# jonnylaw/bayesian_dlms

Measured on AMD Instinct MI355X. Metric: Kalman filter+smooth series*timesteps/sec, higher is better.
Workload: dtype f64

## Files before the change

### bayesian_dlms_amd/_lib.py

```python
import ctypes
import os

HERE = os.path.dirname(os.path.abspath(__file__))
LIB_PATH = os.environ.get("DLM_ENGINE_LIB") or os.path.join(HERE, "libdlm_engine.so")

DLM_MEM_DEVICE, DLM_MEM_HOST = 0, 1
OPT_SMOOTHER_COMPAT_Q1 = 1 << 0
OPT_SVD_RAW_W_Q2 = 1 << 1
OPT_SVD_SAMPLER_Q9 = 1 << 2
OPT_FORCE_GENERIC = 1 << 3
OPT_STATS_OUTER = 1 << 4
OPT_ASYNC = 1 << 5
OPT_FFBS_SIMSMOOTH = 1 << 6
OPT_PACKED_SYM = 1 << 7
OPT_MODEL_UNCHANGED = 1 << 8
OPT_COUNT_STEPS = 1 << 9
OPT_TRUST_MODEL_UNCHANGED = 1 << 10
OPT_LOGLIK_LITERAL_Q7 = 1 << 11
OPT_STUDENTT_LITERAL = 1 << 12
OPT_NO_LANE = 1 << 16
OPT_NO_SAMPLER16 = 1 << 17
OPT_NO_WAVE = 1 << 18
OPT_FORCE_WAVE = 1 << 19
OPT_NO_SPARSE_F = 1 << 20
OPT_NO_SMALL_BATCH = 1 << 21
OPT_NO_STEADY = 1 << 22
OPT_NO_PIPE = 1 << 23
OPT_SHARED_COV = 1 << 24
OPT_SVD_PER_SERIES = 1 << 25
OPT_SAMPLER_PER_SERIES = 1 << 26
OPT_DRAW_EIG = 1 << 27
OPT_SMOOTHER_PER_SERIES = 1 << 28
OPT_NO_TABLE_REUSE = 1 << 29
OPT_TEST_FAIL_AFTER_TABLES = 1 << 30
# ... 107 lines not shown
```

### bayesian_dlms_amd/csrc/dlm_engine.hip

```cpp
#include "../../include/dlm_engine.h"
#include <cstdlib>
#include "dlm_internal.h"

#include <rccl/rccl.h>

#include <cstdio>
#include <cstring>
#include <set>
#include <string>
#include <vector>

using dlm::KArgs;

struct Workspace {
  void* p = nullptr;
  size_t bytes = 0;
  Workspace* next;
  explicit Workspace(Workspace*& list) : next(list) { list = this; }
};
template <class T>
struct Ws : Workspace {
  using Workspace::Workspace;
  operator T*() const { return (T*)p; }
};
// ... 420 lines not shown
int start_sampler_normals(dlm_engine* e, const KArgs& k, dlm::SampTabs& tb, bool big, hipEvent_t gate) {
  if (!k.z) {
    int rc = ensure(e, e->zws, big ? dlm::wave48_sampler_shared_normals_bytes(k) : dlm::sampler_shared_normals_bytes(k));
    if (rc) return rc;
    if (!e->rng_stream) {
      HIP_TRY(e, hipStreamCreateWithFlags(&e->rng_stream, hipStreamNonBlocking));
      HIP_TRY(e, hipEventCreateWithFlags(&e->rng_ev, hipEventDisableTiming));
    }
    if ((rc = aux_fork(e, e->rng_stream, e->rng_busy, gate, false))) return rc;
    if (big) HIP_TRY(e, dlm::launch_wave48_sampler_shared_normals(k, e->zws, e->rng_stream));
    else HIP_TRY(e, dlm::launch_sampler_shared_normals(k, e->zws, e->rng_stream));
    tb.z4 = e->zws;
  }
  return DLM_OK;
}
int start_rts_tables(dlm_engine* e, const KArgs& k, dlm::RtsTabs& tb) {
  bool fresh = false;
  int rc = ensure(e, e->rtsws, dlm::rts_shared_ws_bytes(k), &fresh);
  if (rc) return rc;
  if (fresh) HIP_TRY(e, hipMemsetAsync(e->rtsws, 0, 64, e->stream));
  if ((rc = ensure(e, e->covws, sizeof(double) * dlm::covtabs_doubles(k.d, k.T)))) return rc;
  if ((rc = ensure_route(e, (size_t)k.N)) || (rc = ensure_cov_stream(e))) return rc;
  dlm::RtsKeep keep{};
  dlm::rts_shared_carve(e->rtsws, k, tb, keep);
  dlm::CovTabs ctb{};
  dlm::covtabs_carve(e->covws, k.d, k.T, ctb);
  const bool no_reuse = (k.flags & DLM_OPT_NO_TABLE_REUSE) != 0;
  const int* gate = keep.ctl + dlm::RTS_CTL_GATE;
  e->rts_last = true;
  HIP_TRY(e, dlm::launch_rts_shared_mark(k, e->route, tb, e->stream));
  HIP_TRY(e, dlm::launch_rts_key_check(k, e->sparse_k, e->sp_dev, keep, no_reuse, e->stream));
  HIP_TRY(e, dlm::launch_rts_shared_cov(k, e->sparse_k, e->sp_dev, tb, ctb, gate, e->stream));
  if ((rc = aux_fork(e, e->cov_stream, e->cov_busy, e->cov_ev[0]))) return rc;
  HIP_TRY(e, dlm::launch_rts_shared_tables(k, e->sparse_k, e->sp_dev, tb, gate, e->cov_stream));
  HIP_TRY(e, dlm::launch_rts_key_commit(k, e->sparse_k, e->sp_dev, keep, no_reuse, e->cov_stream));
  return DLM_OK;
}
int ensure_shared(dlm_engine* e, const KArgs& k, dlm::CovTabs& tb, bool with_backward) {
  int rc = ensure(e, e->covws, sizeof(double) * dlm::covtabs_doubles(k.d, k.T));
  if (rc || (rc = ensure_route(e, (size_t)k.N)) || (rc = ensure_side(e, k.N, k.T)) || (rc = ensure_cov_stream(e))) return rc;
  dlm::covtabs_carve(e->covws, k.d, k.T, tb);
// ... 557 lines not shown
  if ((rc = st.commit())) return rc;
  if ((rc = analyse_g(e, k, model->G, opts->mem == DLM_MEM_HOST))) return rc;
  if (want_packed && (rc = packed_path(e, k))) return rc;
  bool fused_fast = fast_smoother_ok(e, k) || use_tiled(k);
  if (want_packed) k.packed = 3;
  const bool q1 = (k.flags & DLM_OPT_SMOOTHER_COMPAT_Q1) != 0;
  const bool rts_shared = fast_shape_ok(k) && e->sparse_k > 0 && !use_lane(k) && !k.packed && !(k.flags & DLM_OPT_SHARED_COV) &&
                          (q1 ? !fused_fast : fast_smoother_ok(e, k)) && dlm::rts_shared_eligible(k, !q1);
  if (!filt) {
    k.packed |= (fast_smoother_ok(e, k) && e->sparse_k > 0 && !use_lane(k) && !rts_shared) ? 1 : 0;
    if ((rc = ensure(e, e->fws, (k.packed & 1) ? N * (T + 1) * (size_t)dlm::packed_rec_bytes((int)d) : N * (T + 1) * rec * sizeof(double)))) return rc;
    k.filt = e->fws;
  }
  if ((rc = mark(e, 0))) return rc;
  dlm::RtsTabs rtb{};
  if (rts_shared && (rc = start_rts_tables(e, k, rtb))) return rc;
  if (rts_shared && (k.flags & DLM_OPT_TEST_FAIL_AFTER_TABLES))
    return fail(e, DLM_ERR_UNSUPPORTED, "DLM_OPT_TEST_FAIL_AFTER_TABLES");
  if ((rc = mark_plain(e, k))) return rc;
  if (filt && fast_smoother_ok(e, k) && use_shared_cov(e, k)) {
    dlm::CovTabs tb;
    if ((rc = run_shared_filter(e, k, tb, true))) return rc;
    if ((rc = mark(e, 1))) return rc;
    k.filt_in = k.filt;
    if ((rc = run_shared_smoother(e, k, tb))) return rc;
    if ((rc = mark(e, 2))) return rc;
    return st.finish(opts->flags & DLM_OPT_ASYNC);
  }
  if ((rc = run_filter(e, k, fused_fast))) return rc;
  if (rts_shared && (rc = join_cov(e))) return rc;
  if ((rc = mark(e, 1))) return rc;
  k.filt_in = k.filt;
  if (rts_shared) {
    k.route = e->route; k.route_take = 0;
    e->variant = "sparse16-rts-shared";
    HIP_TRY(e, dlm::launch_rts_shared_means(k, e->sparse_k, e->sp_dev, rtb, q1, e->stream));
    if (!q1) {
      KArgs kg = k;
      kg.route_take = 1;
      HIP_TRY(e, dlm::launch_sparse16_smoother(kg, e->sparse_k, e->sp_dev, e->side, e->stream));
    }
  } else if ((rc = run_smoother(e, k, fused_fast))) return rc;
  if ((rc = mark(e, 2))) return rc;
  return st.finish(opts->flags & DLM_OPT_ASYNC);
// ... 295 lines not shown
```

### bayesian_dlms_amd/csrc/dlm_internal.h

```cpp
#pragma once
#include <hip/hip_runtime.h>
#include <stdint.h>
#include <type_traits>

namespace dlm {

struct KArgs {
  int d, p, T, N;
  const double* F; long long f_stride;
  const double* G; int n_g; const int* g_index; const double* dt;
  const double* V; long long v_stride;
  const double* W; long long w_stride;
  long long v_tstride, w_tstride;
  const double* m0; long long m0_stride;
  const double* C0; long long c0_stride;
  const double* y;
  const double* z;
  const double* filt_in;
  double* filt;
  double* prior;
  double* fq;
  double* smooth;
  double* theta;
  double* cond;
// ... 68 lines not shown
hipError_t launch_sparse16_sampler(const KArgs& a, int K, const SparseT* tabs_dev, hipStream_t s);
hipError_t launch_small_mv_sampler(const KArgs& a, hipStream_t s);
hipError_t launch_sparse16_rts(const KArgs& a, int K, const SparseT* tabs_dev, hipStream_t s);
hipError_t launch_small_mv_rts(const KArgs& a, hipStream_t s);
hipError_t launch_sparse16_smoother(const KArgs& a, int K, const SparseT* cols_dev, const double* side, hipStream_t s);
hipError_t launch_sparse16_count_gaps(const KArgs& a, unsigned char* plain, hipStream_t s);
struct CovTabs {
  double* ftab;
  double* btab;
  double* cside;
  double* eq;
  double* mc;
  double* sc;
  int frow, brow;
  const int* skip;
};
size_t covtabs_doubles(int d, int T);
void covtabs_carve(double* base, int d, int T, CovTabs& t);
bool shared_cov_eligible(const KArgs& a);
hipError_t launch_sparse16_cov_filter(const KArgs& a, int K, const SparseT* rows_dev, const CovTabs& tabs, hipStream_t s);
hipError_t launch_sparse16_cov_smoother(const KArgs& a, int K, const SparseT* cols_dev, const CovTabs& tabs, hipStream_t s);
hipError_t launch_sparse16_mean_filter(const KArgs& a, int K, const SparseT* rows_dev, const CovTabs& tabs, hipStream_t s);
hipError_t launch_sparse16_mean_smoother(const KArgs& a, int K, const SparseT* cols_dev, const CovTabs& tabs, hipStream_t s);

struct SampTabs {
  double* rows;
  double* zrec;
  double* zeros;
  unsigned char* need;
  int* status;
  double* z4;
  int zstride;
  const double* mc4;
// ... 24 lines not shown
constexpr unsigned RTS_KEY_FLAGS = (1u << 0) | (1u << 22);
struct RtsKeySrc {
  int d, T, K;
  unsigned flags;
  const double *F, *V, *W, *C0;
  const SparseT* sp;
};
enum { RTS_CTL_HIT = 10,
       RTS_CTL_GATE = 11,
       RTS_CTL_VALID = 12,
       RTS_CTL_LAST = 13 };
struct RtsKeep { int* ctl; unsigned* key; };
constexpr int RTS_KEY_WORDS = 8 + 2 * (15 + 1 + 2 * 15 * 15) + 2 * (int)(sizeof(SparseT) / 4);
bool rts_shared_eligible(const KArgs& a, bool textbook);
size_t rts_shared_ws_bytes(const KArgs& a);
void rts_shared_carve(void* ws, const KArgs& a, RtsTabs& tb, RtsKeep& keep);
hipError_t launch_rts_key_check(const KArgs& a, int K, const SparseT* tabs_dev, const RtsKeep& keep, bool no_reuse, hipStream_t s);
hipError_t launch_rts_key_commit(const KArgs& a, int K, const SparseT* tabs_dev, const RtsKeep& keep, bool no_reuse, hipStream_t s);
hipError_t launch_rts_shared_cov(const KArgs& a, int K, const SparseT* tabs_dev, RtsTabs& tb, const CovTabs& ctb, const int* gate, hipStream_t s);
hipError_t launch_rts_shared_tables(const KArgs& a, int K, const SparseT* tabs_dev, const RtsTabs& tb, const int* gate, hipStream_t s);
hipError_t launch_rts_shared_mark(const KArgs& a, unsigned char* route, const RtsTabs& tb, hipStream_t s);
hipError_t launch_rts_shared_means(const KArgs& a, int K, const SparseT* tabs_dev, const RtsTabs& tb, bool own_rts, hipStream_t s);

bool wave48_sampler_shared_model_ok(const KArgs& a);
bool wave48_sampler_shared_eligible(const KArgs& a);
size_t wave48_sampler_shared_ws_bytes(const KArgs& a);
void wave48_sampler_shared_carve(void* ws, const KArgs& a, SampTabs& tb);
hipError_t launch_wave48_sampler_shared_tables(const KArgs& a, const SampTabs& tb, hipStream_t s, hipEvent_t after_filter = nullptr);
hipError_t launch_wave48_sampler_shared_draw(const KArgs& a, const SampTabs& tb, hipStream_t s);
size_t wave48_ktab_doubles(const KArgs& a);
hipError_t launch_wave48_steady_filter(const KArgs& a, const double* ktab, const int* settle, hipStream_t s);
// ... 159 lines not shown
```

### bayesian_dlms_amd/csrc/dlm_sampler16.hip

```cpp
#include "dlm_internal.h"
#include "dlm_wave.h"
#include "../../include/dlm_engine.h"

namespace dlm {
namespace s16 {

constexpr int IL = 17;
constexpr int IMG = 16 * IL;

__device__ __forceinline__ d4 mm(const d4& x, const d4& y, int rows) {
  d4 acc = {0.0, 0.0, 0.0, 0.0};
#pragma unroll
  for (int r = 0; r < 4; ++r)
    if (4 * r < rows) acc = __builtin_amdgcn_mfma_f64_16x16x4f64(x[r], y[r], acc, 0, 0, 0);
  return acc;
}
__device__ __forceinline__ void to_img(const d4& x, double* img, int g, int c) {
#pragma unroll
  for (int r = 0; r < 4; ++r) img[(4 * r + g) * IL + c] = x[r];
}
__device__ __forceinline__ d4 transposed(const d4& x, double* img, int g, int c) {
  to_img(x, img, g, c);
  wave_sync();
  d4 y;
// ... 1137 lines not shown
}

#ifndef DLM_RTS_SHARED_MIN
#define DLM_RTS_SHARED_MIN 2048
#endif
#ifndef DLM_RTS_SHARED_MIN_TEXTBOOK
#define DLM_RTS_SHARED_MIN_TEXTBOOK 6144
#endif
bool rts_shared_eligible(const KArgs& a, bool textbook) {
  return sampler_shared_model_ok(a) && a.y && !(a.flags & (DLM_OPT_FORCE_GENERIC | DLM_OPT_SMOOTHER_PER_SERIES | DLM_OPT_NO_STEADY)) &&
         (a.N >= (textbook ? DLM_RTS_SHARED_MIN_TEXTBOOK : DLM_RTS_SHARED_MIN) || (a.flags & DLM_OPT_NO_SMALL_BATCH));
}
static size_t rts_key_bytes() { return up64((size_t)RTS_KEY_WORDS * 4); }
size_t rts_shared_ws_bytes(const KArgs& a) {
  const size_t n1 = (size_t)a.T + 1, rec = (size_t)a.d + (size_t)a.d * a.d;
  return 64 + rts_key_bytes() + up64(n1 * s16::RJ_ROW * 8) + up64(n1 * rec * 8) + up64(n1);
}
void rts_shared_carve(void* ws, const KArgs& a, RtsTabs& tb, RtsKeep& keep) {
  const size_t n1 = (size_t)a.T + 1, rec = (size_t)a.d + (size_t)a.d * a.d;
  char* p = (char*)ws;
  keep.ctl = (int*)p; p += 64;
  keep.key = (unsigned*)p; p += rts_key_bytes();
  tb.jrows = (double*)p; p += up64(n1 * s16::RJ_ROW * 8);
  tb.srec = (double*)p;  p += up64(n1 * rec * 8);
  tb.need = (unsigned char*)p;
  tb.status = keep.ctl; tb.gaps = tb.status + 8; tb.skip = tb.status + 9;
  tb.crec = nullptr; tb.crec_stride = 0;
}
static RtsKeySrc rts_key_of(const KArgs& a, int K, const SparseT* tabs_dev) {
  RtsKeySrc s;
  s.d = a.d; s.T = a.T; s.K = K; s.flags = a.flags & RTS_KEY_FLAGS;
  s.F = a.F; s.V = a.V; s.W = a.W; s.C0 = a.C0; s.sp = tabs_dev;
  return s;
}
hipError_t launch_rts_key_check(const KArgs& a, int K, const SparseT* tabs_dev, const RtsKeep& keep, bool no_reuse, hipStream_t s) {
  if (a.d < 1 || a.d > 15) return hipErrorInvalidValue;
  return launch(s16::k_rts_key_check, dim3(1), dim3(256), 0, s, rts_key_of(a, K, tabs_dev), (const unsigned*)keep.key, keep.ctl, no_reuse ? 1 : 0);
}
hipError_t launch_rts_key_commit(const KArgs& a, int K, const SparseT* tabs_dev, const RtsKeep& keep, bool no_reuse, hipStream_t s) {
  if (a.d < 1 || a.d > 15) return hipErrorInvalidValue;
// ... 69 lines not shown
```

### bayesian_dlms_amd/csrc/dlm_sparse16.hip

```cpp
#include "dlm_internal.h"
#include "dlm_wave.h"
#include "../../include/dlm_engine.h"

namespace dlm {

constexpr int LD = 17;
constexpr int IMG = 16 * LD;
constexpr int WAVE_LDS = 2 * IMG + 8 * 16 + 2;

#ifndef DLM_SM_WAVES
#define DLM_SM_WAVES 4
#endif
#ifndef DLM_FI_WAVES
#define DLM_FI_WAVES 5
#endif
#ifndef DLM_SM_WAVES_K2
#define DLM_SM_WAVES_K2 5
#endif
constexpr int SM_WAVES_K2 = DLM_SM_WAVES_K2;
constexpr int SM_WAVES = DLM_SM_WAVES, FI_WAVES = DLM_FI_WAVES;

#ifdef DLM_STAMP
#define STAMP(k) { const unsigned long long _t = stamp(); seg[k] += _t - tlast; tlast = _t; }
#else
// ... 377 lines not shown
    } else {
      cc = R;
      steady = false;
      settle_reset(settle);
      bst128(rside, offS, (t + 1) * 16, __builtin_nan(""), __builtin_nan(""));
    }
    if (fq && lane == 0) { fq[2 * (t + 1)] = f; fq[2 * (t + 1) + 1] = Q; }
    const int so = (t + 1) * recb;
#pragma unroll
    for (int r = 0; r < 4; ++r) bst(rout, offA[r], so, cc[r]);
    wave_sync();
  }
  if (LL && a.loglik && lane == 0) a.loglik[n] = ll;
  if (!COV && a.counters && lane == 0) {
    if (nsteady) atomicAdd(&a.counters[0], (unsigned long long)nsteady);
    if (a.route) atomicAdd(&a.counters[3], 1ull);
  }
  bool bad = false;
#pragma unroll
  for (int r = 0; r < 4; ++r) bad |= va[r] && !isfinite(cc[r]);
  if (__ballot(bad) != 0ull) st |= DLM_ST_NONFINITE;
  if (a.status && lane == 0 && st) atomicOr(&a.status[n], st);
}

template <int K, bool SIM, bool IRR, bool LL = false>
__global__ __launch_bounds__(256, SIM ? 4 : FI_WAVES) void k_filter_sp16(KArgs a, const SparseT* __restrict__ sp,
                                                     double* __restrict__ side, double* __restrict__ xplus) {
  __shared__ __attribute__((aligned(16))) double lds[4 * WAVE_LDS + (SIM ? 4 * IMG : 0)];
  filter_body<K, SIM, IRR, LL>(a, sp, side, xplus, lds);
}
template <int K>
__global__ __launch_bounds__(64) void k_cov_filter_sp16(KArgs a, const SparseT* __restrict__ sp, double* __restrict__ side,
                                                        double* __restrict__ kftab, const int* __restrict__ skip) {
  if (skip && *skip) return;
  __shared__ __attribute__((aligned(16))) double lds[4 * WAVE_LDS];
  __builtin_amdgcn_s_setprio(3);
  filter_body<K, false, false, false, true>(a, sp, side, nullptr, lds, kftab);
}

__global__ __launch_bounds__(64) void k_cov_fill_sp16(double* __restrict__ ftab, int rowd, double* __restrict__ cside, const int* __restrict__ settle, int T) {
  const int t = blockIdx.x, ts = settle[0];
  if (t <= ts || t > T) return;
  const double* src = ftab + (size_t)ts * rowd;
  double* dst = ftab + (size_t)t * rowd;
  for (int i = threadIdx.x; i < rowd; i += 64) dst[i] = src[i];
  if (threadIdx.x < 2) cside[2 * (size_t)t + threadIdx.x] = cside[2 * (size_t)ts + threadIdx.x];
}

constexpr int SM_LDS = 2 * IMG + 3 * 16 + 2;
template <int K, bool IRR, bool PIPE = false, bool COV = false, bool PLAIN = false>
__device__ __forceinline__ void smoother_body(const KArgs& a, const SparseT* __restrict__ sp, const double* __restrict__ side,
                                              double* lds , char* ring_all, double* __restrict__ kbtab = nullptr) {
  const int lane = threadIdx.x & 63;
  const int wave = __builtin_amdgcn_readfirstlane(threadIdx.x >> 6);
  const int n = blockIdx.x * (int)(blockDim.x >> 6) + wave;
// ... 486 lines not shown
  if (__ballot(vc && !isfinite(thn)) != 0ull) st |= DLM_ST_NONFINITE;
  if (a.stats) {
    const int L = stats_len(d, 1, a.flags);
    double* sout = a.stats + (size_t)n * L;
    if (lane == 0) { sout[0] = ssy; sout[1] = nob; sout[L - 1] = (double)T; }
    if (outer) {
#pragma unroll
      for (int r = 0; r < 4; ++r) { const int i = 4 * r + g; if (i < d && vc) sout[2 + i + c * d] = so[r]; }
    } else if (g == 0 && vc) sout[2 + c] = ssc;
  }
  if (a.status && lane == 0 && st) atomicOr(&a.status[n], st);
}


constexpr int MEAN4_LDS = 6 * 64;
constexpr int MEAN_AHEAD = 8;

template <int K, int NP, int MODE>
__global__ __launch_bounds__(256) void k_mean_filter_sp16(KArgs a, const SparseT* __restrict__ sp, CovTabs tb) {
  constexpr bool REC = MODE != 0, CMP = MODE != 1;
  constexpr int NS = (REC ? NP : 0) + (CMP ? 1 : 0);
  __shared__ __attribute__((aligned(16))) double lds[4 * MEAN4_LDS];
  extern __shared__ __attribute__((aligned(16))) char ring_all[];
  const int lane = threadIdx.x & 63;
  const int wave = __builtin_amdgcn_readfirstlane(threadIdx.x >> 6);
  const int n0 = 4 * (blockIdx.x * (int)(blockDim.x >> 6) + wave);
  if (n0 >= a.N) return;
  const int j = lane >> 4, c = lane & 15;
  const int nser = a.N - n0 < 4 ? a.N - n0 : 4;
  const bool have = j < nser;
  const int n = have ? n0 + j : n0;
  double* vM = lds + wave * MEAN4_LDS;
  double* vW = vM + 64;
  double* vA = vW + 64;
  double* vH = vA + 64;
  const int d = a.d, T = a.T, rec = d + d * d, recb = rec * 8, frow = recb + 128;
  const bool vc = c < d;
  int idx[K];
  double val[K];
#pragma unroll
  for (int s = 0; s < K; ++s) { idx[s] = 16 * j + sp[0].idx[c][s]; val[s] = sp[0].val[c][s]; }
  const double V = a.V[0];
  const double* m0 = a.m0 + (size_t)n * a.m0_stride;
  const double* y = a.y + (size_t)n * T;
  const size_t sbytes = (size_t)(T + 1) * recb;
  char* bout = REC ? (char*)a.filt + (size_t)n0 * sbytes : nullptr;
  const __amdgpu_buffer_rsrc_t rout = mk_rsrc(bout, REC ? (size_t)nser * sbytes : 0);
  const __amdgpu_buffer_rsrc_t rcmp = mk_rsrc(CMP ? (char*)(tb.mc + (size_t)(n0 / 4) * (T + 1) * 64) : nullptr, CMP ? (size_t)(T + 1) * 512 : 0);
  const int offmc = have ? lane * 8 : OOB;
  double* eqn = tb.eq + (size_t)n * (T + 1);
  const double Fc = vc ? a.F[c] : 0.0;
  double F4[4];
#pragma unroll
  for (int k = 0; k < 4; ++k) F4[k] = ((c & 3) + 4 * k < d) ? a.F[(c & 3) + 4 * k] : 0.0;
  const int npc = rec / 2;
  unsigned psrc[NP];
  int pdst[NP], pser[NP];
#pragma unroll
  for (int k = 0; k < NP; ++k) {
    const int q = 64 * k + lane, sj = q / npc, pp = q - sj * npc;
    pser[k] = sj;
    pdst[k] = sj < nser ? (int)((size_t)sj * sbytes) + pp * 16 : OOB;
    psrc[k] = pp < 8 ? (0x80000000u | (unsigned)((16 * (sj & 3) + 2 * pp) * 8)) : (unsigned)(pp * 16);
  }
  const unsigned vH_lds = lds_addr_of(vH);
  char* ring = ring_all + wave * 2 * frow;
  const unsigned ring_lds = lds_addr_of(ring);
  const unsigned pkf = recb + c * 8, ptd = c * 8;
  const i4 rtab = rsrc_words(tb.ftab, (unsigned)((size_t)(T + 1) * frow));
  const int nrow = frow / 16;
  lds_dma<4>(rtab, ring_lds, 0, lane, nrow);
  lds_dma<4>(rtab, ring_lds + frow, frow, lane, nrow);
  double mcol = vc ? m0[c] : 0.0, mrow = mcol;
  int st = (V > 0.0) ? 0 : DLM_ST_NOT_PD;
  unsigned nsteady = 0;
  bool dead = !have;
  unsigned deadmask = (unsigned)(0xf << nser) & 0xf;
  vM[lane] = mcol; vW[lane] = mrow;
  double yk[4];
#pragma unroll
  for (int k = 0; k < 4; ++k) yk[k] = (16 * k + c < T) ? y[16 * k + c] : 0.0;
  asm volatile("" ::"v"(yk[0]), "v"(yk[1]), "v"(yk[2]), "v"(yk[3]));
  double ek[4] = {__builtin_nan(""), 0.0, 0.0, 0.0};
  wave_sync();
  vm_wait<1>();

  auto store = [&](const d2 (&pc)[NP], int so) {
#pragma unroll
    for (int k = 0; k < NP; ++k) bst128(rout, ((deadmask >> pser[k]) & 1u) ? OOB : pdst[k], so, pc[k]);
  };
  if constexpr (REC) {
    d2 pc[NP];
    {
      double td = lds_read64<0>(ring_lds + ptd);
      asm volatile("s_waitcnt lgkmcnt(0)" : "+v"(td)::"memory");
      vH[lane] = vc ? mcol : td;
      wave_sync();
#pragma unroll
      for (int k = 0; k < NP; ++k) pc[k] = lds_read128((psrc[k] & 0x80000000u) ? vH_lds + (psrc[k] & 0x7fffffffu) : ring_lds + psrc[k]);
      lds_wait<NP>(pc);
    }
    lds_dma<4>(rtab, ring_lds, (T >= 2 ? 2 : T) * frow, lane, nrow);
    store(pc, 0);
  } else lds_dma<4>(rtab, ring_lds, (T >= 2 ? 2 : T) * frow, lane, nrow);
  if constexpr (CMP) bst(rcmp, offmc, 0, vc ? mcol : 0.0);
  for (int t = 0; t < T; ++t) {
    if (t > 0 && (t & 63) == 0) {
#pragma unroll
      for (int k = 0; k < 4; ++k) yk[k] = (t + 16 * k + c < T) ? y[t + 16 * k + c] : 0.0;
      asm volatile("" ::"v"(yk[0]), "v"(yk[1]), "v"(yk[2]), "v"(yk[3]));
    }
    const int kk = (t >> 4) & 3;
    const double yt = row_pick(kk == 0 ? yk[0] : kk == 1 ? yk[1] : kk == 2 ? yk[2] : yk[3], lane, t & 15);
    if (!dead && !(yt == yt)) {
      dead = true;
      if (c == 0) a.route[n] = 1;
    }
    deadmask = 0;
#pragma unroll
    for (int q = 0; q < 4; ++q) deadmask |= (__builtin_amdgcn_readlane((int)dead, 16 * q) & 1) << q;
    if (deadmask == 0xfu) break;
    if (t == 0) vm_wait<NS + 1>(); else vm_wait<2 * NS + 1>();
    const unsigned slot = ring_lds + ((t + 1) & 1) * frow;
    double kfc = lds_read64<0>(slot + pkf);
    asm volatile("s_waitcnt lgkmcnt(0)" : "+v"(kfc)::"memory");
    const double rqs = readlane_d(kfc, 15);
    const double rq = fabs(rqs);
    double ac = vW[idx[0]] * val[0];
#pragma unroll
    for (int s = 1; s < K; ++s) ac = fma(vW[idx[s]], val[s], ac);
    double e, erq;
    if (rqs < 0.0) {
      nsteady += 4 - __builtin_popcount(deadmask);
      const double f = row_lane0(row_sum(Fc * ac), lane);
      e = yt - f; erq = e * rq;
      mcol = fma(kfc, e, ac);
      mrow = mcol;
    } else {
      double ar = vM[idx[0]] * val[0];
#pragma unroll
      for (int s = 1; s < K; ++s) ar = fma(vM[idx[s]], val[s], ar);
      vA[lane] = ac;
      wave_sync();
      double pf = 0.0;
#pragma unroll
      for (int k = 0; k < 4; ++k) pf = fma(vA[16 * j + (c & 3) + 4 * k], F4[k], pf);
      pf = pf + dpp_mov<0xB1>(pf);
      const double f = pf + dpp_mov<0x4E>(pf);
      e = yt - f; erq = e * rq;
      mcol = fma(kfc, erq, ac);
      mrow = fma(kfc * rq, e, ar);
    }
    {
      const int k1 = ((t + 1) >> 4) & 3;
      const bool mine = c == ((t + 1) & 15);
      ek[0] = (mine && k1 == 0) ? erq : ek[0]; ek[1] = (mine && k1 == 1) ? erq : ek[1];
      ek[2] = (mine && k1 == 2) ? erq : ek[2]; ek[3] = (mine && k1 == 3) ? erq : ek[3];
      if (((t + 1) & 63) == 63 || t + 1 == T) {
        const int base = (t + 1) & ~63;
#pragma unroll
        for (int k = 0; k < 4; ++k) if (!dead && base + 16 * k + c <= t + 1) eqn[base + 16 * k + c] = ek[k];
      }
    }
    wave_sync();
    vM[lane] = vc ? mcol : 0.0; vW[lane] = vc ? mrow : 0.0;
    wave_sync();
    if constexpr (REC) {
      d2 pc[NP];
      {
        double td = lds_read64<0>(slot + ptd);
        asm volatile("s_waitcnt lgkmcnt(0)" : "+v"(td)::"memory");
        vH[lane] = vc ? mcol : td;
        wave_sync();
#pragma unroll
        for (int k = 0; k < NP; ++k) pc[k] = lds_read128((psrc[k] & 0x80000000u) ? vH_lds + (psrc[k] & 0x7fffffffu) : slot + psrc[k]);
        lds_wait<NP>(pc);
      }
      { const int tn = t + 3 <= T ? t + 3 : T; lds_dma<4>(rtab, slot, tn * frow, lane, nrow); }
      store(pc, (t + 1) * recb);
    } else { const int tn = t + 3 <= T ? t + 3 : T; lds_dma<4>(rtab, slot, tn * frow, lane, nrow); }
    if constexpr (CMP) bst(rcmp, dead ? OOB : offmc, (t + 1) * 512, vc ? mcol : 0.0);
  }
  vm_wait<0>();
  if (have && !dead && c == 0) a.route[n] = 0;
  if (a.counters && lane == 0) { atomicAdd(&a.counters[2], (unsigned long long)(4 - __builtin_popcount(deadmask))); if (nsteady) atomicAdd(&a.counters[0], (unsigned long long)nsteady); }
  const unsigned long long badl = __ballot(!dead && vc && !isfinite(mcol));
  if (have && !dead && c == 0) {
    const int sj = st | (((badl >> (16 * j)) & 0xffffull) ? DLM_ST_NONFINITE : 0);
    if (a.status && sj) atomicOr(&a.status[n], sj);
  }
}

template <int K, int NP, bool REC>
__global__ __launch_bounds__(256) void k_mean_smoother_sp16(KArgs a, const SparseT* __restrict__ sp, CovTabs tb) {
  constexpr int NS = REC ? NP : 1;
  __shared__ __attribute__((aligned(16))) double lds[4 * MEAN4_LDS];
  extern __shared__ __attribute__((aligned(16))) char ring_all[];
  const int lane = threadIdx.x & 63;
  const int wave = __builtin_amdgcn_readfirstlane(threadIdx.x >> 6);
  const int n0 = 4 * (blockIdx.x * (int)(blockDim.x >> 6) + wave);
// ... 147 lines not shown
  }
  vm_wait<0>();
  if (a.counters && lane == 0 && nsteady) atomicAdd(&a.counters[1], (unsigned long long)nsteady);
  const unsigned long long badl = __ballot(!dead && vc && !isfinite(sm));
  if (!dead && c == 0) {
    const int sj = st | (((badl >> (16 * j)) & 0xffffull) ? DLM_ST_NONFINITE : 0);
    if (a.status && sj) atomicOr(&a.status[n], sj);
  }
}

size_t covtabs_doubles(int d, int T) { return (size_t)(T + 1) * (3 * (size_t)(d + d * d) + 16 + 16 + 2) + 64; }
void covtabs_carve(double* base, int d, int T, CovTabs& t) {
  const size_t rec = (size_t)(d + d * d), n1 = (size_t)T + 1;
  t.frow = (int)(rec * 8 + 128); t.brow = (int)(2 * rec * 8 + 128);
  t.ftab = base; t.btab = t.ftab + n1 * (rec + 16); t.cside = t.btab + n1 * (2 * rec + 16);
  t.skip = nullptr;
}
bool shared_cov_eligible(const KArgs& a) {
  return a.d <= 15 && a.p == 1 && !a.g_index && !a.dt && !a.f_stride && !a.v_tstride && !a.w_tstride && !a.v_stride && !a.w_stride &&
         !a.c0_stride && !a.packed && !a.prior && !a.fq && !a.loglik && a.filt && (a.flags & DLM_OPT_SHARED_COV) && !(a.flags & DLM_OPT_FORCE_GENERIC) &&
         4 * ((size_t)a.T + 1) * (size_t)(a.d + a.d * a.d) * 8 < ((size_t)1 << 31);
}

int sparse16_analyse(const double* G , int d, SparseT* rows, SparseT* cols) {
  int kmax = 1;
  for (int pass = 0; pass < 2; ++pass) {
    SparseT* t = pass ? cols : rows;
    for (int j = 0; j < 16; ++j)
      for (int s = 0; s < 4; ++s) { t->idx[j][s] = 0; t->val[j][s] = 0.0; }
    for (int j = 0; j < d; ++j) {
      int cnt = 0;
      for (int l = 0; l < d; ++l) {
        const double v = pass ? G[l + j * d]  : G[j + l * d] ;
        if (v != 0.0) {
          if (cnt == 4) return 99;
          t->idx[j][cnt] = l; t->val[j][cnt] = v; ++cnt;
// ... 57 lines not shown
}

hipError_t launch_sparse16_simsmooth(const KArgs& a, int K, const SparseT* tabs_dev, const double* side,
                                     const double* xplus, hipStream_t s) {
  return pick<1, 2, 3, 4>(K, [&](auto k) { return launch_ss<k()>(a, tabs_dev, side, xplus, s); });
}

static KArgs cov_args(const KArgs& a, const CovTabs& tb) {
  KArgs k = a;
  k.N = 1; k.y = nullptr; k.status = nullptr; k.route = nullptr; k.counters = nullptr; k.loglik = nullptr; k.prior = nullptr; k.fq = nullptr;
  k.filt = tb.ftab; k.filt_in = tb.ftab; k.smooth = tb.btab; k.packed = 0; k.m0_stride = 0; k.plain = nullptr;
  return k;
}
template <int K>
static hipError_t launch_cf(const KArgs& a, const SparseT* sp, const CovTabs& tb, hipStream_t s) {
  int* settle = (int*)(tb.cside + 2 * ((size_t)a.T + 1));
  hipError_t err = hipMemsetD32Async((hipDeviceptr_t)settle, a.T, 1, s);
  if (err != hipSuccess) return err;
  KArgs k = cov_args(a, tb);
  k.settle_step = (a.flags & DLM_OPT_NO_STEADY) ? nullptr : settle;
  if ((err = launch(k_cov_filter_sp16<K>, dim3(1), dim3(64), 0, s, k, sp, tb.cside, tb.ftab + (a.d + a.d * a.d), tb.skip)) != hipSuccess) return err;
  return launch(k_cov_fill_sp16, dim3(a.T + 1), dim3(64), 0, s, tb.ftab, tb.frow / 8, tb.cside, (const int*)settle, a.T);
}
template <int K>
static hipError_t launch_cs(const KArgs& a, const SparseT* sp, const CovTabs& tb, hipStream_t s) {
  const size_t ring = 2 * ((size_t)(a.d + a.d * a.d) * 8 + 16);
  return launch(k_cov_smoother_sp16<K>, dim3(1), dim3(64), ring, s, cov_args(a, tb), sp, (const double*)tb.cside, tb.btab);
}
template <class F>
static hipError_t with_mean_np(int d, F f) { return pick<4, 6, 8>(d <= 10 ? 4 : d <= 13 ? 6 : 8, f); }
template <int K>
static hipError_t launch_mf(const KArgs& a, const SparseT* sp, const CovTabs& tb, hipStream_t s) {
  const int wpb = a.N < 8192 ? 1 : 4, nw = (a.N + 3) / 4;
  const dim3 grid((nw + wpb - 1) / wpb), blk(64 * wpb);
  const size_t ring = (size_t)wpb * 2 * tb.frow;
  return pick<0, 2, 1>(tb.mc ? (a.filt ? 2 : 0) : 1, [&](auto MODE) {
    return with_mean_np(a.d, [&](auto NP) { return launch(k_mean_filter_sp16<K, NP(), decltype(MODE)::value>, grid, blk, ring, s, a, sp, tb); });
// ... 31 lines not shown
```

### include/dlm_engine.h

```cpp
#ifndef DLM_ENGINE_H
#define DLM_ENGINE_H

#include <stdint.h>

#ifdef __cplusplus
extern "C" {
#endif

typedef struct dlm_engine dlm_engine;

enum {
  DLM_OK = 0,
  DLM_ERR_ARG = -1,
  DLM_ERR_HIP = -2,
  DLM_ERR_UNSUPPORTED = -3,
  DLM_ERR_RCCL = -4
};

enum { DLM_MEM_DEVICE = 0, DLM_MEM_HOST = 1 };

enum {
  DLM_OPT_SMOOTHER_COMPAT_Q1 = 1u << 0,
  DLM_OPT_SVD_RAW_W_Q2 = 1u << 1,
  DLM_OPT_SVD_SAMPLER_Q9 = 1u << 2,
  DLM_OPT_FORCE_GENERIC = 1u << 3,
  DLM_OPT_STATS_OUTER = 1u << 4,
  DLM_OPT_ASYNC = 1u << 5,
  DLM_OPT_FFBS_SIMSMOOTH = 1u << 6,
  DLM_OPT_PACKED_SYM = 1u << 7,
  DLM_OPT_MODEL_UNCHANGED = 1u << 8,
  DLM_OPT_COUNT_STEPS = 1u << 9,
  DLM_OPT_TRUST_MODEL_UNCHANGED = 1u << 10,
  DLM_OPT_LOGLIK_LITERAL_Q7 = 1u << 11,
  DLM_OPT_STUDENTT_LITERAL = 1u << 12,
  DLM_OPT_NO_LANE = 1u << 16,
  DLM_OPT_NO_SAMPLER16 = 1u << 17,
  DLM_OPT_NO_WAVE = 1u << 18,
  DLM_OPT_FORCE_WAVE = 1u << 19,
  DLM_OPT_NO_SPARSE_F = 1u << 20,
  DLM_OPT_NO_SMALL_BATCH = 1u << 21,
  DLM_OPT_NO_STEADY = 1u << 22,
  DLM_OPT_NO_PIPE = 1u << 23,
  DLM_OPT_SVD_PER_SERIES = 1u << 25,
  DLM_OPT_SAMPLER_PER_SERIES = 1u << 26,
  DLM_OPT_DRAW_EIG = 1u << 27,
  DLM_OPT_SMOOTHER_PER_SERIES = 1u << 28,
  DLM_OPT_NO_TABLE_REUSE = 1u << 29,
  DLM_OPT_TEST_FAIL_AFTER_TABLES = 1u << 30,
  DLM_OPT_SHARED_COV = 1u << 24
// ... 135 lines not shown
```

### integration/scala/Batched.scala

```scala
package com.github.jonnylaw.dlm.gpu

import java.nio.{ByteBuffer, ByteOrder, DoubleBuffer}
import breeze.linalg.{DenseMatrix, DenseVector}
import com.github.jonnylaw.dlm._

final class Native private[gpu] () {
  @native def engineCreate(device: Int): Long
  @native def engineDestroy(h: Long): Unit
  @native def lastError(h: Long): String
  @native def version(): String
  @native def lastVariant(h: Long): String
  @native def engineSetStream(h: Long, stream: Long): Unit
  @native def engineSync(h: Long): Unit
  @native def engineWaitStream(h: Long, stream: Long): Unit
  @native def streamWaitEngine(h: Long, stream: Long): Unit
  @native def lastTiming(h: Long): Array[Double]
  @native def lastCounters(h: Long): Array[Long]
  @native def lastTableReuse(h: Long): Int
  @native def address(directBuffer: java.nio.Buffer): Long
  @native def bufferAlloc(h: Long, bytes: Long): Long
  @native def bufferFree(h: Long, dev: Long): Unit
  @native def bufferUpload(h: Long, dstDev: Long, dstOffset: Long, srcHost: Long, bytes: Long): Unit
  @native def bufferDownload(h: Long, srcDev: Long, srcOffset: Long, dstHost: Long, bytes: Long): Unit
  @native def bufferFill(h: Long, dstDev: Long, dstOffset: Long, byteValue: Int, bytes: Long): Unit
// ... 29 lines not shown
  val SvdSamplerQ9 = 1 << 2
  val ForceGeneric = 1 << 3
  val StatsOuter = 1 << 4
  val FfbsSimSmooth = 1 << 6
  val PackedSym = 1 << 7
  val ModelUnchanged = 1 << 8
  val CountSteps = 1 << 9
  val LoglikLiteralQ7 = 1 << 11
  val StudenttLiteral = 1 << 12
  val TrustModelUnchanged = 1 << 10
  val SvdPerSeries = 1 << 25
  val SamplerPerSeries = 1 << 26
  val DrawEig = 1 << 27
  val SmootherPerSeries = 1 << 28
  val NoTableReuse = 1 << 29
  val NoSteady = 1 << 22
  val LiteralReference = SmootherCompatQ1 | SvdRawWQ2 | SvdSamplerQ9
}

final class DeviceBuffer private[gpu] (owner: Batched, val bytes: Long) {
  private[gpu] var ptr: Long = Native.lib.bufferAlloc(owner.handle, bytes)
  def free(): Unit = if (ptr != 0L) { Native.lib.bufferFree(owner.handle, ptr); ptr = 0L }
}

final class Batched(device: Int = 0, stagingBytes: Int = 64 << 20) extends AutoCloseable {
  private val nat = Native.lib
  private[gpu] val handle: Long = nat.engineCreate(device)
  private val staging: ByteBuffer = ByteBuffer.allocateDirect(stagingBytes).order(ByteOrder.nativeOrder)
  private val stagingAddr: Long = nat.address(staging)
  def close(): Unit = nat.engineDestroy(handle)
// ... 277 lines not shown
```

Measured before the change: 1.297 billion.

## Route shared-RTS forward pass through mean-only filter using shared covariance tables

```diff
diff --git a/bayesian_dlms_amd/_lib.py b/bayesian_dlms_amd/_lib.py
--- a/bayesian_dlms_amd/_lib.py
+++ b/bayesian_dlms_amd/_lib.py
@@ -18,6 +18,7 @@
 OPT_TRUST_MODEL_UNCHANGED = 1 << 10
 OPT_LOGLIK_LITERAL_Q7 = 1 << 11
 OPT_STUDENTT_LITERAL = 1 << 12
+OPT_FORWARD_PER_SERIES = 1 << 13
 OPT_NO_LANE = 1 << 16
 OPT_NO_SAMPLER16 = 1 << 17
 OPT_NO_WAVE = 1 << 18
diff --git a/bayesian_dlms_amd/csrc/dlm_engine.hip b/bayesian_dlms_amd/csrc/dlm_engine.hip
--- a/bayesian_dlms_amd/csrc/dlm_engine.hip
+++ b/bayesian_dlms_amd/csrc/dlm_engine.hip
@@ -458,17 +458,14 @@
   }
   return DLM_OK;
 }
-int start_rts_tables(dlm_engine* e, const KArgs& k, dlm::RtsTabs& tb) {
+int start_rts_tables(dlm_engine* e, const KArgs& k, dlm::RtsTabs& tb, dlm::CovTabs& ctb) {
   bool fresh = false;
   int rc = ensure(e, e->rtsws, dlm::rts_shared_ws_bytes(k), &fresh);
   if (rc) return rc;
   if (fresh) HIP_TRY(e, hipMemsetAsync(e->rtsws, 0, 64, e->stream));
-  if ((rc = ensure(e, e->covws, sizeof(double) * dlm::covtabs_doubles(k.d, k.T)))) return rc;
   if ((rc = ensure_route(e, (size_t)k.N)) || (rc = ensure_cov_stream(e))) return rc;
   dlm::RtsKeep keep{};
-  dlm::rts_shared_carve(e->rtsws, k, tb, keep);
-  dlm::CovTabs ctb{};
-  dlm::covtabs_carve(e->covws, k.d, k.T, ctb);
+  dlm::rts_shared_carve(e->rtsws, k, tb, keep, ctb);
   const bool no_reuse = (k.flags & DLM_OPT_NO_TABLE_REUSE) != 0;
   const int* gate = keep.ctl + dlm::RTS_CTL_GATE;
   e->rts_last = true;
@@ -1056,7 +1053,8 @@
   }
   if ((rc = mark(e, 0))) return rc;
   dlm::RtsTabs rtb{};
-  if (rts_shared && (rc = start_rts_tables(e, k, rtb))) return rc;
+  dlm::CovTabs rctb{};
+  if (rts_shared && (rc = start_rts_tables(e, k, rtb, rctb))) return rc;
   if (rts_shared && (k.flags & DLM_OPT_TEST_FAIL_AFTER_TABLES))
     return fail(e, DLM_ERR_UNSUPPORTED, "DLM_OPT_TEST_FAIL_AFTER_TABLES");
   if ((rc = mark_plain(e, k))) return rc;
@@ -1069,7 +1067,16 @@
     if ((rc = mark(e, 2))) return rc;
     return st.finish(opts->flags & DLM_OPT_ASYNC);
   }
-  if ((rc = run_filter(e, k, fused_fast))) return rc;
+  if (rts_shared && !(k.flags & DLM_OPT_FORWARD_PER_SERIES) && dlm::mean_filter_fits(k)) {
+    if (fused_fast && (rc = ensure_side(e, k.N, k.T))) return rc;
+    KArgs kf = k;
+    kf.route = e->route; kf.route_take = 0;
+    rctb.eq = nullptr; rctb.mc = nullptr; rctb.marked = 1;
+    e->variant = "sparse16";
+    HIP_TRY(e, dlm::launch_sparse16_mean_filter(kf, e->sparse_k, e->sp_dev, rctb, e->stream));
+    kf.route_take = 2;
+    HIP_TRY(e, dlm::launch_sparse16_filter(kf, e->sparse_k, e->sp_dev, fused_fast ? (double*)e->side : nullptr, nullptr, e->stream));
+  } else if ((rc = run_filter(e, k, fused_fast))) return rc;
   if (rts_shared && (rc = join_cov(e))) return rc;
   if ((rc = mark(e, 1))) return rc;
   k.filt_in = k.filt;
diff --git a/bayesian_dlms_amd/csrc/dlm_internal.h b/bayesian_dlms_amd/csrc/dlm_internal.h
--- a/bayesian_dlms_amd/csrc/dlm_internal.h
+++ b/bayesian_dlms_amd/csrc/dlm_internal.h
@@ -106,9 +106,12 @@
   double* sc;
   int frow, brow;
   const int* skip;
-};
+  int marked;
+};
+__host__ __device__ inline int* covtabs_settle(const CovTabs& t, int T) { return (int*)(t.cside + 2 * ((size_t)T + 1)); }
 size_t covtabs_doubles(int d, int T);
 void covtabs_carve(double* base, int d, int T, CovTabs& t);
+bool mean_filter_fits(const KArgs& a);
 bool shared_cov_eligible(const KArgs& a);
 hipError_t launch_sparse16_cov_filter(const KArgs& a, int K, const SparseT* rows_dev, const CovTabs& tabs, hipStream_t s);
 hipError_t launch_sparse16_cov_smoother(const KArgs& a, int K, const SparseT* cols_dev, const CovTabs& tabs, hipStream_t s);
@@ -163,7 +166,7 @@
 constexpr int RTS_KEY_WORDS = 8 + 2 * (15 + 1 + 2 * 15 * 15) + 2 * (int)(sizeof(SparseT) / 4);
 bool rts_shared_eligible(const KArgs& a, bool textbook);
 size_t rts_shared_ws_bytes(const KArgs& a);
-void rts_shared_carve(void* ws, const KArgs& a, RtsTabs& tb, RtsKeep& keep);
+void rts_shared_carve(void* ws, const KArgs& a, RtsTabs& tb, RtsKeep& keep, CovTabs& ctb);
 hipError_t launch_rts_key_check(const KArgs& a, int K, const SparseT* tabs_dev, const RtsKeep& keep, bool no_reuse, hipStream_t s);
 hipError_t launch_rts_key_commit(const KArgs& a, int K, const SparseT* tabs_dev, const RtsKeep& keep, bool no_reuse, hipStream_t s);
 hipError_t launch_rts_shared_cov(const KArgs& a, int K, const SparseT* tabs_dev, RtsTabs& tb, const CovTabs& ctb, const int* gate, hipStream_t s);
diff --git a/bayesian_dlms_amd/csrc/dlm_sampler16.hip b/bayesian_dlms_amd/csrc/dlm_sampler16.hip
--- a/bayesian_dlms_amd/csrc/dlm_sampler16.hip
+++ b/bayesian_dlms_amd/csrc/dlm_sampler16.hip
@@ -1175,16 +1175,21 @@
 static size_t rts_key_bytes() { return up64((size_t)RTS_KEY_WORDS * 4); }
 size_t rts_shared_ws_bytes(const KArgs& a) {
   const size_t n1 = (size_t)a.T + 1, rec = (size_t)a.d + (size_t)a.d * a.d;
-  return 64 + rts_key_bytes() + up64(n1 * s16::RJ_ROW * 8) + up64(n1 * rec * 8) + up64(n1);
-}
-void rts_shared_carve(void* ws, const KArgs& a, RtsTabs& tb, RtsKeep& keep) {
+  return 64 + rts_key_bytes() + up64(n1 * s16::RJ_ROW * 8) + up64(n1 * rec * 8) + up64(n1) +
+         up64(n1 * (rec + 16) * 8) + up64((2 * n1 + 64) * 8);
+}
+void rts_shared_carve(void* ws, const KArgs& a, RtsTabs& tb, RtsKeep& keep, CovTabs& ctb) {
   const size_t n1 = (size_t)a.T + 1, rec = (size_t)a.d + (size_t)a.d * a.d;
   char* p = (char*)ws;
   keep.ctl = (int*)p; p += 64;
   keep.key = (unsigned*)p; p += rts_key_bytes();
   tb.jrows = (double*)p; p += up64(n1 * s16::RJ_ROW * 8);
   tb.srec = (double*)p;  p += up64(n1 * rec * 8);
-  tb.need = (unsigned char*)p;
+  tb.need = (unsigned char*)p; p += up64(n1);
+  ctb = CovTabs{};
+  ctb.frow = (int)(rec * 8 + 128);
+  ctb.ftab = (double*)p; p += up64(n1 * (rec + 16) * 8);
+  ctb.cside = (double*)p;
   tb.status = keep.ctl; tb.gaps = tb.status + 8; tb.skip = tb.status + 9;
   tb.crec = nullptr; tb.crec_stride = 0;
 }
diff --git a/bayesian_dlms_amd/csrc/dlm_sparse16.hip b/bayesian_dlms_amd/csrc/dlm_sparse16.hip
--- a/bayesian_dlms_amd/csrc/dlm_sparse16.hip
+++ b/bayesian_dlms_amd/csrc/dlm_sparse16.hip
@@ -415,7 +415,7 @@
   if (LL && a.loglik && lane == 0) a.loglik[n] = ll;
   if (!COV && a.counters && lane == 0) {
     if (nsteady) atomicAdd(&a.counters[0], (unsigned long long)nsteady);
-    if (a.route) atomicAdd(&a.counters[3], 1ull);
+    if (a.route && a.route_take != 2) atomicAdd(&a.counters[3], 1ull);
   }
   bool bad = false;
 #pragma unroll
@@ -435,11 +435,14 @@
                                                         double* __restrict__ kftab, const int* __restrict__ skip) {
   if (skip && *skip) return;
   __shared__ __attribute__((aligned(16))) double lds[4 * WAVE_LDS];
+  if (threadIdx.x == 0) *(int*)(side + 2 * ((size_t)a.T + 1)) = a.T;
   __builtin_amdgcn_s_setprio(3);
   filter_body<K, false, false, false, true>(a, sp, side, nullptr, lds, kftab);
 }
 
-__global__ __launch_bounds__(64) void k_cov_fill_sp16(double* __restrict__ ftab, int rowd, double* __restrict__ cside, const int* __restrict__ settle, int T) {
+__global__ __launch_bounds__(64) void k_cov_fill_sp16(double* __restrict__ ftab, int rowd, double* __restrict__ cside, const int* __restrict__ settle, int T,
+                                                      const int* __restrict__ skip) {
+  if (skip && *skip) return;
   const int t = blockIdx.x, ts = settle[0];
   if (t <= ts || t > T) return;
   const double* src = ftab + (size_t)ts * rowd;
@@ -956,6 +959,10 @@
 
 
 constexpr int MEAN4_LDS = 6 * 64;
+__device__ __forceinline__ int covtabs_settle_row(const CovTabs& tb, int T) {
+  const int ts = __builtin_amdgcn_readfirstlane(*covtabs_settle(tb, T));
+  return ts < 0 ? 0 : ts > T ? T : ts;
+}
 constexpr int MEAN_AHEAD = 8;
 
 template <int K, int NP, int MODE>
@@ -972,6 +979,11 @@
   const int nser = a.N - n0 < 4 ? a.N - n0 : 4;
   const bool have = j < nser;
   const int n = have ? n0 + j : n0;
+  bool dead = !have || (tb.marked && a.route[n] != 0);
+  unsigned deadmask = 0;
+#pragma unroll
+  for (int q = 0; q < 4; ++q) deadmask |= (__builtin_amdgcn_readlane((int)dead, 16 * q) & 1) << q;
+  if (deadmask == 0xfu) return;
   double* vM = lds + wave * MEAN4_LDS;
   double* vW = vM + 64;
   double* vA = vW + 64;
@@ -990,7 +1002,9 @@
   const __amdgpu_buffer_rsrc_t rout = mk_rsrc(bout, REC ? (size_t)nser * sbytes : 0);
   const __amdgpu_buffer_rsrc_t rcmp = mk_rsrc(CMP ? (char*)(tb.mc + (size_t)(n0 / 4) * (T + 1) * 64) : nullptr, CMP ? (size_t)(T + 1) * 512 : 0);
   const int offmc = have ? lane * 8 : OOB;
-  double* eqn = tb.eq + (size_t)n * (T + 1);
+  const bool weq = tb.eq != nullptr;
+  double* eqn = weq ? tb.eq + (size_t)n * (T + 1) : nullptr;
+  const int tset = covtabs_settle_row(tb, T);
   const double Fc = vc ? a.F[c] : 0.0;
   double F4[4];
 #pragma unroll
@@ -1016,8 +1030,6 @@
   double mcol = vc ? m0[c] : 0.0, mrow = mcol;
   int st = (V > 0.0) ? 0 : DLM_ST_NOT_PD;
   unsigned nsteady = 0;
-  bool dead = !have;
-  unsigned deadmask = (unsigned)(0xf << nser) & 0xf;
   vM[lane] = mcol; vW[lane] = mrow;
   double yk[4];
 #pragma unroll
@@ -1045,15 +1057,15 @@
     lds_dma<4>(rtab, ring_lds, (T >= 2 ? 2 : T) * frow, lane, nrow);
     store(pc, 0);
   } else lds_dma<4>(rtab, ring_lds, (T >= 2 ? 2 : T) * frow, lane, nrow);
-  if constexpr (CMP) bst(rcmp, offmc, 0, vc ? mcol : 0.0);
-  for (int t = 0; t < T; ++t) {
+  if constexpr (CMP) bst(rcmp, dead ? OOB : offmc, 0, vc ? mcol : 0.0);
+  auto observe = [&](int t, double& yt) -> bool {
     if (t > 0 && (t & 63) == 0) {
 #pragma unroll
       for (int k = 0; k < 4; ++k) yk[k] = (t + 16 * k + c < T) ? y[t + 16 * k + c] : 0.0;
       asm volatile("" ::"v"(yk[0]), "v"(yk[1]), "v"(yk[2]), "v"(yk[3]));
     }
     const int kk = (t >> 4) & 3;
-    const double yt = row_pick(kk == 0 ? yk[0] : kk == 1 ? yk[1] : kk == 2 ? yk[2] : yk[3], lane, t & 15);
+    yt = row_pick(kk == 0 ? yk[0] : kk == 1 ? yk[1] : kk == 2 ? yk[2] : yk[3], lane, t & 15);
     if (!dead && !(yt == yt)) {
       dead = true;
       if (c == 0) a.route[n] = 1;
@@ -1061,24 +1073,51 @@
     deadmask = 0;
 #pragma unroll
     for (int q = 0; q < 4; ++q) deadmask |= (__builtin_amdgcn_readlane((int)dead, 16 * q) & 1) << q;
-    if (deadmask == 0xfu) break;
+    return deadmask != 0xfu;
+  };
+  auto advance = [&]() {
+    double ac = vW[idx[0]] * val[0];
+#pragma unroll
+    for (int s = 1; s < K; ++s) ac = fma(vW[idx[s]], val[s], ac);
+    return ac;
+  };
+  auto steady_step = [&](double ac, double kfc, double rq, double yt) {
+    nsteady += 4 - __builtin_popcount(deadmask);
+    const double f = row_lane0(row_sum(Fc * ac), lane);
+    const double e = yt - f;
+    mcol = fma(kfc, e, ac);
+    mrow = mcol;
+    return e * rq;
+  };
+  auto put_eq = [&](int t, double erq) {
+    const int k1 = ((t + 1) >> 4) & 3;
+    const bool mine = c == ((t + 1) & 15);
+    ek[0] = (mine && k1 == 0) ? erq : ek[0]; ek[1] = (mine && k1 == 1) ? erq : ek[1];
+    ek[2] = (mine && k1 == 2) ? erq : ek[2]; ek[3] = (mine && k1 == 3) ? erq : ek[3];
+    if (((t + 1) & 63) == 63 || t + 1 == T) {
+      const int base = (t + 1) & ~63;
+#pragma unroll
+      for (int k = 0; k < 4; ++k) if (!dead && base + 16 * k + c <= t + 1) eqn[base + 16 * k + c] = ek[k];
+    }
+  };
+  d2 pc[REC ? NP : 1];
+  double td = 0.0, kfc = 0.0, rq = 0.0;
+  bool frozen = false;
+  int t = 0;
+  for (; t < T && !frozen; ++t) {
+    double yt;
+    if (!observe(t, yt)) break;
     if (t == 0) vm_wait<NS + 1>(); else vm_wait<2 * NS + 1>();
     const unsigned slot = ring_lds + ((t + 1) & 1) * frow;
-    double kfc = lds_read64<0>(slot + pkf);
+    kfc = lds_read64<0>(slot + pkf);
     asm volatile("s_waitcnt lgkmcnt(0)" : "+v"(kfc)::"memory");
     const double rqs = readlane_d(kfc, 15);
-    const double rq = fabs(rqs);
-    double ac = vW[idx[0]] * val[0];
-#pragma unroll
-    for (int s = 1; s < K; ++s) ac = fma(vW[idx[s]], val[s], ac);
-    double e, erq;
-    if (rqs < 0.0) {
-      nsteady += 4 - __builtin_popcount(deadmask);
-      const double f = row_lane0(row_sum(Fc * ac), lane);
-      e = yt - f; erq = e * rq;
-      mcol = fma(kfc, e, ac);
-      mrow = mcol;
-    } else {
+    rq = fabs(rqs);
+    frozen = rqs < 0.0 && t + 1 >= tset;
+    const double ac = advance();
+    double erq;
+    if (rqs < 0.0) erq = steady_step(ac, kfc, rq, yt);
+    else {
       double ar = vM[idx[0]] * val[0];
 #pragma unroll
       for (int s = 1; s < K; ++s) ar = fma(vM[idx[s]], val[s], ar);
@@ -1089,43 +1128,56 @@
       for (int k = 0; k < 4; ++k) pf = fma(vA[16 * j + (c & 3) + 4 * k], F4[k], pf);
       pf = pf + dpp_mov<0xB1>(pf);
       const double f = pf + dpp_mov<0x4E>(pf);
-      e = yt - f; erq = e * rq;
+      const double e = yt - f;
+      erq = e * rq;
       mcol = fma(kfc, erq, ac);
       mrow = fma(kfc * rq, e, ar);
     }
-    {
-      const int k1 = ((t + 1) >> 4) & 3;
-      const bool mine = c == ((t + 1) & 15);
-      ek[0] = (mine && k1 == 0) ? erq : ek[0]; ek[1] = (mine && k1 == 1) ? erq : ek[1];
-      ek[2] = (mine && k1 == 2) ? erq : ek[2]; ek[3] = (mine && k1 == 3) ? erq : ek[3];
-      if (((t + 1) & 63) == 63 || t + 1 == T) {
-        const int base = (t + 1) & ~63;
-#pragma unroll
-        for (int k = 0; k < 4; ++k) if (!dead && base + 16 * k + c <= t + 1) eqn[base + 16 * k + c] = ek[k];
-      }
-    }
+    if (weq) put_eq(t, erq);
     wave_sync();
     vM[lane] = vc ? mcol : 0.0; vW[lane] = vc ? mrow : 0.0;
     wave_sync();
+    const int tn = t + 3 <= T ? t + 3 : T;
     if constexpr (REC) {
-      d2 pc[NP];
-      {
-        double td = lds_read64<0>(slot + ptd);
-        asm volatile("s_waitcnt lgkmcnt(0)" : "+v"(td)::"memory");
+      td = lds_read64<0>(slot + ptd);
+      asm volatile("s_waitcnt lgkmcnt(0)" : "+v"(td)::"memory");
+      vH[lane] = vc ? mcol : td;
+      wave_sync();
+#pragma unroll
+      for (int k = 0; k < NP; ++k) pc[k] = lds_read128((psrc[k] & 0x80000000u) ? vH_lds + (psrc[k] & 0x7fffffffu) : slot + psrc[k]);
+      lds_wait<NP>(pc);
+      if (!frozen) lds_dma<4>(rtab, slot, tn * frow, lane, nrow);
+      store(pc, (t + 1) * recb);
+    } else if (!frozen) lds_dma<4>(rtab, slot, tn * frow, lane, nrow);
+    if constexpr (CMP) bst(rcmp, dead ? OOB : offmc, (t + 1) * 512, vc ? mcol : 0.0);
+  }
+  if (frozen) {
+    vm_wait<0>();
+    for (; t < T; ++t) {
+      double yt;
+      if (!observe(t, yt)) break;
+      const double ac = advance();
+      const double erq = steady_step(ac, kfc, rq, yt);
+      if (weq) put_eq(t, erq);
+      wave_sync();
+      vW[lane] = vc ? mrow : 0.0;
+      if constexpr (REC) {
         vH[lane] = vc ? mcol : td;
         wave_sync();
 #pragma unroll
-        for (int k = 0; k < NP; ++k) pc[k] = lds_read128((psrc[k] & 0x80000000u) ? vH_lds + (psrc[k] & 0x7fffffffu) : slot + psrc[k]);
+        for (int k = 0; k < NP; ++k) if (psrc[k] & 0x80000000u) pc[k] = lds_read128(vH_lds + (psrc[k] & 0x7fffffffu));
         lds_wait<NP>(pc);
-      }
-      { const int tn = t + 3 <= T ? t + 3 : T; lds_dma<4>(rtab, slot, tn * frow, lane, nrow); }
-      store(pc, (t + 1) * recb);
-    } else { const int tn = t + 3 <= T ? t + 3 : T; lds_dma<4>(rtab, slot, tn * frow, lane, nrow); }
-    if constexpr (CMP) bst(rcmp, dead ? OOB : offmc, (t + 1) * 512, vc ? mcol : 0.0);
+        store(pc, (t + 1) * recb);
+      } else wave_sync();
+      if constexpr (CMP) bst(rcmp, dead ? OOB : offmc, (t + 1) * 512, vc ? mcol : 0.0);
+    }
   }
   vm_wait<0>();
-  if (have && !dead && c == 0) a.route[n] = 0;
-  if (a.counters && lane == 0) { atomicAdd(&a.counters[2], (unsigned long long)(4 - __builtin_popcount(deadmask))); if (nsteady) atomicAdd(&a.counters[0], (unsigned long long)nsteady); }
+  if (!tb.marked && have && !dead && c == 0) a.route[n] = 0;
+  if (a.counters && lane == 0) {
+    if (!tb.marked) atomicAdd(&a.counters[2], (unsigned long long)(4 - __builtin_popcount(deadmask)));
+    if (nsteady) atomicAdd(&a.counters[0], (unsigned long long)nsteady);
+  }
   const unsigned long long badl = __ballot(!dead && vc && !isfinite(mcol));
   if (have && !dead && c == 0) {
     const int sj = st | (((badl >> (16 * j)) & 0xffffull) ? DLM_ST_NONFINITE : 0);
@@ -1303,12 +1355,15 @@
   const size_t rec = (size_t)(d + d * d), n1 = (size_t)T + 1;
   t.frow = (int)(rec * 8 + 128); t.brow = (int)(2 * rec * 8 + 128);
   t.ftab = base; t.btab = t.ftab + n1 * (rec + 16); t.cside = t.btab + n1 * (2 * rec + 16);
-  t.skip = nullptr;
+  t.skip = nullptr; t.marked = 0;
+}
+bool mean_filter_fits(const KArgs& a) {
+  return 4 * ((size_t)a.T + 1) * (size_t)(a.d + a.d * a.d) * 8 < ((size_t)1 << 31);
 }
 bool shared_cov_eligible(const KArgs& a) {
   return a.d <= 15 && a.p == 1 && !a.g_index && !a.dt && !a.f_stride && !a.v_tstride && !a.w_tstride && !a.v_stride && !a.w_stride &&
          !a.c0_stride && !a.packed && !a.prior && !a.fq && !a.loglik && a.filt && (a.flags & DLM_OPT_SHARED_COV) && !(a.flags & DLM_OPT_FORCE_GENERIC) &&
-         4 * ((size_t)a.T + 1) * (size_t)(a.d + a.d * a.d) * 8 < ((size_t)1 << 31);
+         mean_filter_fits(a);
 }
 
 int sparse16_analyse(const double* G , int d, SparseT* rows, SparseT* cols) {
@@ -1396,13 +1451,12 @@
 }
 template <int K>
 static hipError_t launch_cf(const KArgs& a, const SparseT* sp, const CovTabs& tb, hipStream_t s) {
-  int* settle = (int*)(tb.cside + 2 * ((size_t)a.T + 1));
-  hipError_t err = hipMemsetD32Async((hipDeviceptr_t)settle, a.T, 1, s);
-  if (err != hipSuccess) return err;
+  int* settle = covtabs_settle(tb, a.T);
+  hipError_t err;
   KArgs k = cov_args(a, tb);
   k.settle_step = (a.flags & DLM_OPT_NO_STEADY) ? nullptr : settle;
   if ((err = launch(k_cov_filter_sp16<K>, dim3(1), dim3(64), 0, s, k, sp, tb.cside, tb.ftab + (a.d + a.d * a.d), tb.skip)) != hipSuccess) return err;
-  return launch(k_cov_fill_sp16, dim3(a.T + 1), dim3(64), 0, s, tb.ftab, tb.frow / 8, tb.cside, (const int*)settle, a.T);
+  return launch(k_cov_fill_sp16, dim3(a.T + 1), dim3(64), 0, s, tb.ftab, tb.frow / 8, tb.cside, (const int*)settle, a.T, tb.skip);
 }
 template <int K>
 static hipError_t launch_cs(const KArgs& a, const SparseT* sp, const CovTabs& tb, hipStream_t s) {
diff --git a/include/dlm_engine.h b/include/dlm_engine.h
--- a/include/dlm_engine.h
+++ b/include/dlm_engine.h
@@ -33,6 +33,7 @@
   DLM_OPT_TRUST_MODEL_UNCHANGED = 1u << 10,
   DLM_OPT_LOGLIK_LITERAL_Q7 = 1u << 11,
   DLM_OPT_STUDENTT_LITERAL = 1u << 12,
+  DLM_OPT_FORWARD_PER_SERIES = 1u << 13,
   DLM_OPT_NO_LANE = 1u << 16,
   DLM_OPT_NO_SAMPLER16 = 1u << 17,
   DLM_OPT_NO_WAVE = 1u << 18,
diff --git a/integration/scala/Batched.scala b/integration/scala/Batched.scala
--- a/integration/scala/Batched.scala
+++ b/integration/scala/Batched.scala
@@ -67,6 +67,7 @@
   val DrawEig = 1 << 27
   val SmootherPerSeries = 1 << 28
   val NoTableReuse = 1 << 29
+  val ForwardPerSeries = 1 << 13
   val NoSteady = 1 << 22
   val LiteralReference = SmootherCompatQ1 | SvdRawWQ2 | SvdSamplerQ9
 }
```

Result: slower. 1.284 billion (-1.0%).
